# ndming/GS-2M

Measured on AMD Instinct MI355X. Metric: train views/s (fwd+bwd raster) at 1M Gaussians 1080p, higher is better.
Workload: dtype f32; 1 GPU; BASELINE configs[2] (c3): 1000000 synthetic Gaussians (SH deg 3), 1 camera 1920x1080 per GPU, feature_count=9, fwd+bwd at the op boundary; gaussians=1000000, visible=844909, num_rendered=2709460, width=1920, height=1080, feature_count=9, parallelism=view-parallel x1, views_per_rank=1

## Files before the change

### gs-2m_amd/csrc/api.hip

```cpp
#include "raster_args.h"
#include <atomic>
#include <mutex>
#include <chrono>
#include <dlfcn.h>

namespace {

constexpr int kLandSlots = 64, kLandWords = 16;
struct LandRing {
    uint32_t* host = nullptr;
    uint32_t* dev = nullptr;
    std::atomic<uint32_t> next{0};
    std::atomic<uint32_t> gen[kLandSlots];
};
LandRing g_land[64];
std::mutex g_land_mutex;
thread_local uint64_t t_last_token = 0;
thread_local long long t_rows_hint = -1;
thread_local long long t_units_hint = -1, t_units_from_token = -1;

static_assert(GS2M_NUM_STAGES == 10, "stage table");
enum Stage { ST_PREPROCESS = 0, ST_UNUSED1, ST_SCAN, ST_EMIT, ST_TILE_SORT, ST_LISTS, ST_BLEND_FWD, ST_UNUSED7,
             ST_BLEND_BWD, ST_GAUSSIAN_BWD, ST_COUNT };
constexpr int kMaxRecords = 8192;
struct Prof {
    std::atomic<int> mode{0};
    int n = 0;
    hipEvent_t ev[kMaxRecords][2];
    int stage[kMaxRecords];
    int created = 0;
    int every = 1;
    int seen3 = 0;
};
Prof g_prof;
std::mutex g_prof_mutex;
std::atomic<int> g_reference_binning{0};
std::atomic<int> g_spin_wait{1};
std::atomic<int> g_debug{0};
std::atomic<int> g_markers{0};

const char* const kStageNames[ST_COUNT] = {"preprocess", "-", "scan", "emit", "tile_sort", "depth_order+quad_lists", "blend_fwd", "-", "blend_bwd", "gaussian_bwd"};

struct Roctx {
    int (*push)(const char*) = nullptr;
    int (*pop)() = nullptr;
    bool tried = false;
    void load() {
        if (tried) return;
        tried = true;
        void* h = dlopen("libroctx64.so", RTLD_NOW | RTLD_GLOBAL);
        if (!h) h = dlopen("libroctx64.so.4", RTLD_NOW | RTLD_GLOBAL);
        if (!h) return;
        push = (int (*)(const char*))dlsym(h, "roctxRangePushA");
        pop = (int (*)())dlsym(h, "roctxRangePop");
    }
};
Roctx g_roctx;

struct StageTimer {
    hipStream_t s;
    int slot = -1;
    int stage;
    int* failed;
    bool marked = false;
    StageTimer(int stage_, hipStream_t s_, int* failed_ = nullptr) : s(s_), stage(stage_), failed(failed_) {
        if (g_markers.load(std::memory_order_relaxed)) {
            g_roctx.load();
            if (g_roctx.push) { g_roctx.push(kStageNames[stage]); marked = true; }
        }
        const bool blend = stage == ST_BLEND_FWD || stage == ST_BLEND_BWD;
        if (g_prof.mode.load(std::memory_order_relaxed) == 0) return;
        {
            std::lock_guard<std::mutex> lock(g_prof_mutex);
            if (g_prof.mode == 0 || (g_prof.mode == 1 && !blend) || (g_prof.mode == 3 && stage != ST_BLEND_BWD) || g_prof.n >= kMaxRecords) return;
            if (g_prof.mode == 3 && (g_prof.seen3++ % g_prof.every) != 0) return;
            slot = g_prof.n++;
            if (slot >= g_prof.created) {
                (void)hipEventCreate(&g_prof.ev[slot][0]);
                (void)hipEventCreate(&g_prof.ev[slot][1]);
                g_prof.created = slot + 1;
            }
            g_prof.stage[slot] = stage;
        }
        (void)hipEventRecord(g_prof.ev[slot][0], s);
    }
    ~StageTimer() {
        if (slot >= 0) (void)hipEventRecord(g_prof.ev[slot][1], s);
        if (failed && g_debug.load(std::memory_order_relaxed) && *failed == 0) {
            hipError_t e = hipGetLastError();
            if (e == hipSuccess) e = hipStreamSynchronize(s);
            if (e != hipSuccess) *failed = stage + 1;
        }
        if (marked && g_roctx.pop) g_roctx.pop();
    }
};
#define DEBUG_CHECK()                                        \
    do {                                                     \
        if (failed_stage) return GS2M_ERR_STAGE(failed_stage - 1); \
    } while (0)

}

extern "C" {

char* gs2m_prealloc_alloc(size_t bytes, void* user) {
    gs2m_prealloc* p = static_cast<gs2m_prealloc*>(user);
    if (!p) return nullptr;
    p->requested = bytes;
    if (p->ptr && bytes <= p->capacity) return p->ptr;
    p->used_fallback = 1;
    return p->fallback ? p->fallback(bytes, p->fallback_user) : nullptr;
}

const char* gs2m_version(void) { return "gs2m_raster 0.5 (gfx950, round 5)"; }

static int forward_impl(gs2m_alloc_fn geometry_alloc, void* geometry_user, gs2m_alloc_fn binning_alloc, void* binning_user,
                        gs2m_alloc_fn image_alloc, void* image_user, const RasterFrame& f, const float* background, int prefiltered,
                        float* out_color, int* out_radii, int* out_observe, float* out_buffer, void* stream_) {
    hipStream_t s = (hipStream_t)stream_;
    const int reference_binning = g_reference_binning.load(), spin_wait = g_spin_wait.load();
    int failed_stage = 0;
    const unsigned bad = frame_faults(f);
    if (bad & (FRAME_BAD_SHAPE | FRAME_BAD_INPUTS)) return GS2M_ERR_INVALID_ARG;
    if (!geometry_alloc || !binning_alloc || !image_alloc || !out_color || !out_buffer || !background) return GS2M_ERR_INVALID_ARG;
    if (f.P > 0 && (!f.opacities || !out_radii || !out_observe)) return GS2M_ERR_INVALID_ARG;
    if (bad & FRAME_BAD_SPLIT_SH) return GS2M_ERR_UNSUPPORTED;
    if (f.P > 0 && f.fc > 0 && !f.features) return GS2M_ERR_INVALID_ARG;
    if (bad & (FRAME_IMAGE_SIDE | FRAME_TILE_COUNT | FRAME_GAUSSIAN_IDS)) return GS2M_ERR_UNSUPPORTED;
    const int P = f.P, width = f.W, height = f.H, tiles_x = f.tiles_x, tiles_y = f.tiles_y;
    const size_t tiles = (size_t)tiles_x * tiles_y, N = (size_t)width * height;

    const size_t Pn = P > 0 ? (size_t)P : 1;
    GeomState gsz = gs2m_carve_geom(nullptr, Pn);
    char* gbase = geometry_alloc(gsz.total_bytes, geometry_user);
    if (!gbase) return GS2M_ERR_ALLOC;
    GeomState g = gs2m_carve_geom(gbase, Pn);

    ImageState isz = gs2m_carve_image(nullptr, N, tiles);
    char* ibase = image_alloc(isz.total_bytes, image_user);
    if (!ibase) return GS2M_ERR_ALLOC;
    ImageState im = gs2m_carve_image(ibase, N, tiles);

    int dev_id = 0;
    HIP_TRY(hipGetDevice(&dev_id));
    if (dev_id < 0 || dev_id >= 64) return GS2M_ERR_UNSUPPORTED;
    LandRing& ring = g_land[dev_id];
    if (!ring.host) {
        std::lock_guard<std::mutex> lock(g_land_mutex);
        if (!ring.host) {
            uint32_t* h = nullptr;
            HIP_TRY(hipHostMalloc((void**)&h, kLandSlots * kLandWords * sizeof(uint32_t), hipHostMallocMapped | hipHostMallocPortable));
            HIP_TRY(hipHostGetDevicePointer((void**)&ring.dev, h, 0));
            for (int k = 0; k < kLandSlots; k++) ring.gen[k] = 0;
            ring.host = h;
        }
    }
    const uint32_t seq = ring.next.fetch_add(1), slot = seq % kLandSlots;
    const uint32_t generation = ring.gen[slot].fetch_add(1) + 1;
    volatile uint32_t* land = ring.host + slot * kLandWords;
    uint32_t* land_dev = ring.dev + slot * kLandWords;
    land[GS2M_LAND_R] = 0xFFFFFFFFu;
    land[GS2M_LAND_HUNITS] = 0xFFFFFFFFu;
    land[GS2M_LAND_PREFILTERED] = 0u;
    land[GS2M_LAND_ROWS] = 0u;
    t_last_token = ((uint64_t)(dev_id + 1) << 40) | ((uint64_t)(generation & 0xFFFFFFFFu) << 8) | slot;

    int R = 0;
    uint32_t U = 0, crowded = GS2M_CROWDED_WAVE;
    if (P > 0) {
        {
            StageTimer t(ST_PREPROCESS, s, &failed_stage);
            ZeroJobs zj = {{g.tile_hist, nullptr, nullptr}, {(size_t)GS2M_HIST_COPIES * GS2M_HIST_COPY_WORDS, 0, 0}};
            gs2m_launch_preprocess(f, out_radii, out_observe, g, reference_binning ? 0 : 1, zj, s);
        }
        if (prefiltered) gs2m_launch_prefiltered_check(P, f.means3D, f.viewmatrix, land_dev + GS2M_LAND_PREFILTERED, s);
        {
            StageTimer t(ST_SCAN, s, &failed_stage);
            gs2m_launch_blockscan(P, g, land_dev, s);
        }
        HIP_TRY(hipGetLastError());
        DEBUG_CHECK();
        if (spin_wait) {
            const auto t0 = std::chrono::steady_clock::now();
            uint32_t spins = 0;
            while (land[GS2M_LAND_R] == 0xFFFFFFFFu || land[GS2M_LAND_HUNITS] == 0xFFFFFFFFu) {
                __builtin_ia32_pause();
                if ((++spins & 0xFFFFu) == 0u && std::chrono::steady_clock::now() - t0 > std::chrono::seconds(2)) break;
            }
        }
        if (land[GS2M_LAND_R] == 0xFFFFFFFFu || land[GS2M_LAND_HUNITS] == 0xFFFFFFFFu) HIP_TRY(hipStreamSynchronize(s));
        if (prefiltered && land[GS2M_LAND_PREFILTERED] != 0u) {
            HIP_TRY(hipStreamSynchronize(s));
            return GS2M_ERR_PREFILTERED;
        }
        if (land[GS2M_LAND_R] >= (1u << 29)) return GS2M_ERR_UNSUPPORTED;
        R = (int)land[GS2M_LAND_R];
        U = land[GS2M_LAND_HUNITS];
        if ((size_t)U * 4 * GS2M_UNIT > (size_t)6 * (size_t)R + 65536) {
            crowded = GS2M_CROWDED_OFF;
            land[GS2M_LAND_R] = 0xFFFFFFFFu;
            land[GS2M_LAND_HUNITS] = 0xFFFFFFFFu;
            gs2m_launch_recount_heavy(P, g, s);
            gs2m_launch_blockscan(P, g, land_dev, s);
            HIP_TRY(hipGetLastError());
            HIP_TRY(hipStreamSynchronize(s));
            if (land[GS2M_LAND_R] != (uint32_t)R) return GS2M_ERR_STAGE(ST_SCAN);
            U = land[GS2M_LAND_HUNITS];
        }
        if (U >= (1u << 22)) return GS2M_ERR_UNSUPPORTED;
    }

    const int tile_bits = (int)higher_msb((uint32_t)tiles);
    const size_t Rn = R > 0 ? (size_t)R : 1;
    const size_t btemp = gs2m_binning_temp_bytes(Rn, tile_bits);
    BinningState bsz = gs2m_carve_binning(nullptr, Rn, btemp, U);
    char* bbase = binning_alloc(bsz.total_bytes, binning_user);
    if (!bbase) return GS2M_ERR_ALLOC;
    BinningState b = gs2m_carve_binning(bbase, Rn, btemp, U);

    if (R > 0) {
        {
            StageTimer t(ST_EMIT, s, &failed_stage);
            ZeroJobs zj = {{nullptr, im.ranges_raw, nullptr}, {0, tiles * 2, 0}};
            gs2m_radix_zero_region(b.temp, (size_t)R, tile_bits, &zj.p[0], &zj.words[0]);
            gs2m_launch_emit(P, width, height, tiles_x, tile_bits, g, b, U, crowded, land_dev, zj, s);
        }
        if (g_debug.load(std::memory_order_relaxed)) {
            uint32_t total = 0;
            HIP_TRY(hipStreamSynchronize(s));
            HIP_TRY(hipMemcpy(&total, g.counters, sizeof(total), hipMemcpyDeviceToHost));
            if (total != (uint32_t)R) return GS2M_ERR_STAGE(ST_EMIT);
        }
        {
            StageTimer t(ST_TILE_SORT, s, &failed_stage);
            HIP_TRY(gs2m_radix_sort_pairs(b.temp, b.temp_bytes, b.keys_unsorted, nullptr, b.sort_keyA, b.sort_valA, b.tile_keys, b.slot_sorted,
                                          (size_t)R, tile_bits, true, s, im.ranges_raw, g.tile_hist));
        }
    } else {
        HIP_TRY(gs2m_zero_async(im.ranges_raw, tiles * 2 * sizeof(uint32_t), s));
        land[GS2M_LAND_ROWS] = 1u;
        if (land[GS2M_LAND_HUNITS] == 0xFFFFFFFFu) land[GS2M_LAND_HUNITS] = 0u;
    }
    DEBUG_CHECK();
    {
        StageTimer t(ST_LISTS, s, &failed_stage);
        gs2m_launch_tile_sort(tiles, tiles_x, tiles_y, (size_t)(R > 0 ? R : 0), b, im, g, s);
    }
    {
        StageTimer t(ST_BLEND_FWD, s, &failed_stage);
        gs2m_launch_blend_fwd_q(width, height, tiles_x, tiles_y, f.fc, background, g, b, im, out_color, out_buffer, out_observe, s);
    }
    DEBUG_CHECK();
    HIP_TRY(hipGetLastError());
    return R;
}

static int backward_impl(const RasterFrame& f, int R, const float* background, const int* radii, char* geom_buffer, char* binning_buffer,
                         char* image_buffer, const float* grad_colors, const float* grad_buffer, const RasterGrads& d,
                         gs2m_alloc_fn scratch_alloc, void* scratch_user, void* stream_) {
    hipStream_t s = (hipStream_t)stream_;
    int failed_stage = 0;
    if (f.P == 0) return GS2M_OK;
    const unsigned bad = frame_faults(f) | grad_faults(f, d);
    if (bad & FRAME_GAUSSIAN_IDS) return GS2M_ERR_UNSUPPORTED;
    if ((bad & (FRAME_BAD_SHAPE | FRAME_NO_GRADS)) || R < 0) return GS2M_ERR_INVALID_ARG;
    if (!geom_buffer || !binning_buffer || !image_buffer || !scratch_alloc || !grad_colors || !radii) return GS2M_ERR_INVALID_ARG;
    if (f.fc > 0 && !grad_buffer) return GS2M_ERR_INVALID_ARG;
    if (bad & FRAME_BAD_SPLIT_SH) return GS2M_ERR_UNSUPPORTED;
    const int P = f.P, width = f.W, height = f.H, tiles_x = f.tiles_x, tiles_y = f.tiles_y, feature_count = f.fc;
    const size_t tiles = (size_t)tiles_x * tiles_y, N = (size_t)width * height;
    const size_t Rn = R > 0 ? (size_t)R : 1;
    GeomState g = gs2m_carve_geom(geom_buffer, (size_t)P);
    BinningState b = gs2m_carve_binning(binning_buffer, Rn, gs2m_binning_temp_bytes(Rn, (int)higher_msb((uint32_t)tiles)), 0);
    ImageState im = gs2m_carve_image(image_buffer, N, tiles);

    const int rowf = gs2m_row_floats(feature_count);
    const long long hint = t_rows_hint;
    long long units = hint >= 0 ? t_units_hint : -1;
// ... 211 lines not shown
```

### gs-2m_amd/csrc/binning.hip

```cpp
#include "common.h"

GeomState gs2m_carve_geom(char* base, size_t P) {
    GeomState g;
    size_t off = base ? (gs2m_align_up((size_t)(uintptr_t)base) - (size_t)(uintptr_t)base) : 0;
    auto take = [&](size_t bytes) {
        char* p = (char*)((uintptr_t)base + off);
        off = gs2m_align_up(off + bytes);
        return p;
    };
    const size_t nb = (P + 255) / 256 + 1, nw = (P + 63) / 64 + 1;
    g.rec = (float4*)take(P * REC_Q * sizeof(float4));
    g.tiles_touched = (uint32_t*)take(P * 4);
    g.rect = (uint2*)take(P * sizeof(uint2));
    g.depth_key = (uint32_t*)take(P * 4);
    g.clamped = (uint8_t*)take(P);
    g.sh_dir = (float*)take(P * 9 * sizeof(float));
    g.counters = (uint32_t*)take(64 * 4);
    g.gauss_rows = (uint32_t*)take(P * 4);
    g.block_tt = (uint32_t*)take(nb * 4);
    g.block_pref = (uint32_t*)take(nb * 4);
    g.block_hu = (uint32_t*)take(nb * 4);
    g.block_hupref = (uint32_t*)take(nb * 4);
    g.wave_rows = (uint32_t*)take(nw * 4);
    g.wave_rowbase = (uint32_t*)take(nw * 4);
// ... 60 lines not shown
    if (lane == 0) s_part[wave] = v;
    gs2m_sync();
    unsigned long long t = 0;
    for (int w = 0; w < nw; w++) t += s_part[w];
    return t;
}

template <typename F>
__device__ __forceinline__ unsigned long long scan_1024_per_block(const uint32_t* __restrict__ in, size_t n, uint32_t* s_w ,
                                                                  unsigned long long* s_part , F emit) {
    const size_t first = (size_t)blockIdx.x * 1024;
    unsigned long long before = 0;
    for (size_t base = 0; base < first; base += 16 * 1024) {
        uint32_t v[16];
#pragma unroll
        for (int k = 0; k < 16; k++) {
            const size_t i = base + (size_t)k * 1024 + threadIdx.x;
            v[k] = i < first ? in[i] : 0u;
        }
#pragma unroll
        for (int k = 0; k < 16; k++) before += v[k];
    }
    const size_t i = first + threadIdx.x;
    const uint32_t mine = i < n ? in[i] : 0u;
    before = block_sum_u64(before, s_part);
    const int lane = threadIdx.x & 63, wave = threadIdx.x >> 6;
    const uint32_t incl = wave_inclusive_scan_u32(mine, lane);
    if (lane == 63) s_w[wave] = incl;
    gs2m_sync();
    uint32_t run = incl - mine, total = 0;
    for (int w = 0; w < 16; w++) {
        if (w < wave) run += s_w[w];
        total += s_w[w];
    }
    if (i < n) emit(i, (uint32_t)before + run, mine);
    return before + total;
}

template <typename F>
__device__ __forceinline__ void scan2_1024_per_block(const uint32_t* __restrict__ in0, const uint32_t* __restrict__ in1, size_t n, uint32_t* s_w ,
                                                     unsigned long long* s_part , F emit, unsigned long long& total0, unsigned long long& total1) {
    const size_t first = (size_t)blockIdx.x * 1024;
    unsigned long long b0 = 0, b1 = 0;
    for (size_t base = 0; base < first; base += 8 * 1024) {
        uint32_t v[8], w[8];
#pragma unroll
        for (int k = 0; k < 8; k++) {
            const size_t i = base + (size_t)k * 1024 + threadIdx.x;
            v[k] = i < first ? in0[i] : 0u;
            w[k] = i < first ? in1[i] : 0u;
        }
#pragma unroll
        for (int k = 0; k < 8; k++) { b0 += v[k]; b1 += w[k]; }
    }
    const size_t i = first + threadIdx.x;
    const uint32_t m0 = i < n ? in0[i] : 0u, m1 = i < n ? in1[i] : 0u;
    const int lane = threadIdx.x & 63, wave = threadIdx.x >> 6;
#pragma unroll
    for (int d = 32; d > 0; d >>= 1) { b0 += __shfl_xor(b0, d, 64); b1 += __shfl_xor(b1, d, 64); }
    const uint32_t i0 = wave_inclusive_scan_u32(m0, lane), i1 = wave_inclusive_scan_u32(m1, lane);
    if (lane == 0) { s_part[wave] = b0; s_part[16 + wave] = b1; }
    if (lane == 63) { s_w[wave] = i0; s_w[16 + wave] = i1; }
    gs2m_sync();
    unsigned long long f0 = 0, f1 = 0;
    uint32_t r0 = i0 - m0, r1 = i1 - m1, t0 = 0, t1 = 0;
    for (int w = 0; w < 16; w++) {
        f0 += s_part[w]; f1 += s_part[16 + w];
        if (w < wave) { r0 += s_w[w]; r1 += s_w[16 + w]; }
        t0 += s_w[w]; t1 += s_w[16 + w];
    }
    if (i < n) emit(i, (uint32_t)f0 + r0, (uint32_t)f1 + r1);
    total0 = f0 + t0;
    total1 = f1 + t1;
}

__global__ void __launch_bounds__(1024) blockscan_kernel(const uint32_t* __restrict__ block_tt, const uint32_t* __restrict__ block_hu, size_t nblocks,
                                                         uint32_t* __restrict__ block_pref, uint32_t* __restrict__ block_hupref,
                                                         uint32_t* __restrict__ counters, uint32_t* landing) {
    __shared__ uint32_t s_w[32];
    __shared__ unsigned long long s_part[32];
    unsigned long long t = 0, u = 0;
    scan2_1024_per_block(block_tt, block_hu, nblocks, s_w, s_part, [&](size_t b, uint32_t e0, uint32_t e1) { block_pref[b] = e0; block_hupref[b] = e1; }, t, u);
    if (blockIdx.x == gridDim.x - 1 && threadIdx.x == 0) {
        const uint32_t r32 = t > 0xFFFFFFFEull ? 0xFFFFFFFEu : (uint32_t)t, u32 = u > 0xFFFFFFFEull ? 0xFFFFFFFEu : (uint32_t)u;
        __hip_atomic_store(reinterpret_cast<unsigned long long*>(landing + GS2M_LAND_R), (unsigned long long)r32 | ((unsigned long long)u32 << 32),
                           __ATOMIC_RELAXED, __HIP_MEMORY_SCOPE_SYSTEM);
        counters[1] = r32;
        counters[GS2M_CNT_HUNITS] = u32;
        counters[GS2M_CNT_SPAN_MID] = 0u;
        counters[GS2M_CNT_SPAN_LONG] = 0u;
    }
}

__global__ void __launch_bounds__(1024) rowscan_kernel(const uint32_t* __restrict__ wave_rows, size_t nwaves, uint32_t* __restrict__ wave_rowbase,
                                                       uint32_t* __restrict__ counters, uint32_t* landing) {
    __shared__ uint32_t s_w[16];
    __shared__ unsigned long long s_part[16];
    const uint32_t heavy_rows = 4u * GS2M_UNIT * counters[GS2M_CNT_HUNITS];
    const unsigned long long total = heavy_rows + scan_1024_per_block(wave_rows, nwaves, s_w, s_part, [&](size_t w, uint32_t excl, uint32_t) { wave_rowbase[w] = heavy_rows + excl; });
    if (blockIdx.x == gridDim.x - 1 && threadIdx.x == 0) {
        counters[GS2M_CNT_ROWS] = (uint32_t)total;
        publish(landing, GS2M_LAND_ROWS, (uint32_t)total + 1u);
    }
}


__device__ __forceinline__ uint2 expand_instance(uint32_t rmin, uint32_t rwid, uint32_t t, const float4 a , const float2 ct ,
                                                 int W, int H, int tiles_x) {
    const uint32_t ry = t / rwid, rx = t - ry * rwid;
    const uint32_t tx = (rmin & 0xFFFFu) + rx, ty = (rmin >> 16) + ry;
    const int px0 = (int)tx * GS2M_TILE, py0 = (int)ty * GS2M_TILE;
    uint32_t mask = gs2m_reaches_quads(a.x, a.y, a.z, a.w, ct.x, ct.y, (float)px0, (float)py0);
    if (px0 + 8 >= W) mask &= 0x5u;
    if (py0 + 8 >= H) mask &= 0x3u;
    return make_uint2(ty * (uint32_t)tiles_x + tx, mask);
}

__global__ void __launch_bounds__(256) emit_kernel(int P, int W, int H, int tiles_x, const uint2* __restrict__ rect,
                                                   const uint32_t* __restrict__ block_pref, const uint32_t* __restrict__ block_hupref,
                                                   const float4* __restrict__ rec,
                                                   const uint32_t* __restrict__ depth_key, uint32_t* __restrict__ keys_out, uint4* __restrict__ e_rec,
                                                   HeavyUnit* __restrict__ hrec,
                                                   uint32_t* __restrict__ gauss_rows, uint32_t* __restrict__ wave_rows,
                                                   uint32_t* __restrict__ counters, uint32_t* __restrict__ tile_hist, int npass, int4 hbits,
                                                   int4 hshift, uint32_t crowded, ZeroJobs zero) {
    __shared__ uint32_t s_th[4][256];
    __shared__ uint32_t s_pref[4][GS2M_WAVE];
    __shared__ uint32_t s_rmin[4][GS2M_WAVE];
    __shared__ uint32_t s_rw[4][GS2M_WAVE];
    __shared__ uint32_t s_off[4][GS2M_WAVE];
    __shared__ uint32_t s_depth[4][GS2M_WAVE];
    __shared__ float4 s_geo[4][GS2M_WAVE];
    __shared__ float2 s_ct[4][GS2M_WAVE];
    __shared__ uint32_t s_rc[4][GS2M_WAVE];
    __shared__ uint32_t s_wtot[4], s_whu[4];
    const int i = blockIdx.x * 256 + threadIdx.x;
    const int wave = threadIdx.x >> 6, lane = threadIdx.x & 63;
    gs2m_zero_jobs(zero, (size_t)i, (size_t)gridDim.x * 256);
#pragma unroll
    for (int p = 0; p < 4; p++) s_th[p][threadIdx.x] = 0u;
    const int hb[4] = {hbits.x, hbits.y, hbits.z, hbits.w}, hs[4] = {hshift.x, hshift.y, hshift.z, hshift.w};
    uint32_t cnt = 0, rmin = 0, rw = 1;
    if (i < P) {
        const uint2 r = rect[i];
        rmin = r.x;
        rw = r.y & 0xFFFFu;
        cnt = rw * (r.y >> 16);
        if (rw == 0u) rw = 1u;
    }
    const bool heavy = gs2m_heavy(cnt, crowded);
    const uint32_t hu = heavy ? (cnt + GS2M_UNIT - 1u) / GS2M_UNIT : 0u;
    const uint32_t incl_all = wave_inclusive_scan_u32(cnt, lane), incl_hu = wave_inclusive_scan_u32(hu, lane);
    if (lane == 63) { s_wtot[wave] = incl_all; s_whu[wave] = incl_hu; }
    const uint32_t lcnt = heavy ? 0u : cnt;
    if (lcnt > 0) {
        const float4* r = rec + (size_t)i * REC_Q;
        s_geo[wave][lane] = r[REC_GEO0];
        s_ct[wave][lane] = make_float2(r[REC_GEO1].x, r[REC_BIN].w);
        s_depth[wave][lane] = depth_key[i];
    }
    const uint32_t incl = wave_inclusive_scan_u32(lcnt, lane);
    const uint32_t total = __shfl(incl, 63, 64);
    s_pref[wave][lane] = incl - lcnt;
    s_rmin[wave][lane] = rmin;
    s_rw[wave][lane] = rw;
    s_rc[wave][lane] = 0u;
    gs2m_sync();
    uint32_t off = block_pref[blockIdx.x], ustart = block_hupref[blockIdx.x];
#pragma unroll
    for (int w = 0; w < 4; w++)
        if (w < wave) { off += s_wtot[w]; ustart += s_whu[w]; }
// ... 147 lines not shown
```

### gs-2m_amd/csrc/common.h

```cpp
#pragma once
#include <hip/hip_runtime.h>
#include <stdint.h>
#include <stddef.h>
#include "../../include/gs2m_raster.h"

typedef float gs2m_v4f __attribute__((ext_vector_type(4)));
template <typename T> __device__ __forceinline__ T gs2m_ldnt(const T* p) { return __builtin_nontemporal_load(p); }
__device__ __forceinline__ float4 gs2m_ldnt(const float4* p) {
    const gs2m_v4f t = __builtin_nontemporal_load(reinterpret_cast<const gs2m_v4f*>(p));
    return make_float4(t.x, t.y, t.z, t.w);
}
template <typename T> __device__ __forceinline__ void gs2m_stnt(T* p, T v) { __builtin_nontemporal_store(v, p); }
__device__ __forceinline__ void gs2m_stnt(float4* p, float4 v) {
    const gs2m_v4f t = {v.x, v.y, v.z, v.w};
    __builtin_nontemporal_store(t, reinterpret_cast<gs2m_v4f*>(p));
}

#define GS2M_ALIGN 256
#define GS2M_WAVE 64

#define REC_Q 8
#define REC_GEO0 0
#define REC_GEO1 1
#define REC_BIN 2
// ... 105 lines not shown
        }
        const size_t rbase = (size_t)blockIdx.x * 11520, rlim = (size_t)P * 45;
        const bool full = rbase + 11520 <= rlim;
        float4 t[12];
        if (full) {
            const float4* g4 = reinterpret_cast<const float4*>(rest + rbase);
#pragma unroll
            for (int i = 0; i < 11; i++) t[i] = gs2m_ldnt(g4 + tid + 256 * i);
            t[11] = tid < 64 ? gs2m_ldnt(g4 + tid + 2816) : make_float4(0.f, 0.f, 0.f, 0.f);
        } else {
#pragma unroll
            for (int i = 0; i < 12; i++) {
                const int k4 = tid + 256 * i;
                const size_t ge = rbase + 4 * (size_t)k4;
                t[i] = make_float4(0.f, 0.f, 0.f, 0.f);
                if (k4 < 2880) {
                    if (ge + 3 < rlim) {
                        t[i] = *reinterpret_cast<const float4*>(rest + ge);
                    } else {
                        if (ge < rlim) t[i].x = rest[ge];
                        if (ge + 1 < rlim) t[i].y = rest[ge + 1];
                        if (ge + 2 < rlim) t[i].z = rest[ge + 2];
                    }
                }
            }
        }
        int row = (4 * tid) / 45, col = 4 * tid - 45 * row;
#pragma unroll
        for (int i = 0; i < 12; i++) {
            if (i < 11 || tid < 64) {
                const float v[4] = {t[i].x, t[i].y, t[i].z, t[i].w};
                int a = row * 49 + 3 + col, left = 45 - col;
#pragma unroll
                for (int c = 0; c < 4; c++) s_sh[a + c + (c >= left ? 4 : 0)] = v[c];
            }
            row += 22; col += 34;
            if (col >= 45) { col -= 45; row += 1; }
        }
    }
}
#endif

GeomState gs2m_carve_geom(char* base, size_t P);
BinningState gs2m_carve_binning(char* base, size_t R, size_t temp_bytes, size_t heavy_units);
size_t gs2m_binning_temp_bytes(size_t R, int tile_bits);
ImageState gs2m_carve_image(char* base, size_t N, size_t tiles);

size_t gs2m_radix_temp_bytes(size_t n, int total_bits);
hipError_t gs2m_radix_sort_pairs(void* temp, size_t temp_bytes, const uint32_t* kin, const uint32_t* vin, uint32_t* kA,
                                 uint32_t* vA, uint32_t* kB, uint32_t* vB, size_t n, int total_bits, bool prezeroed, hipStream_t s,
                                 uint32_t* range_raw = nullptr, const uint32_t* ext_hist = nullptr);
#define GS2M_HIST_COPIES 8
#define GS2M_HIST_COPY_WORDS 1024
void gs2m_radix_plan(int total_bits, int* npass, int bits[4], int shift[4]);
void gs2m_radix_zero_region(void* temp, size_t n, int total_bits, uint32_t** ptr, size_t* words);

#define GS2M_LAND_R 0
#define GS2M_LAND_HUNITS 1
#define GS2M_LAND_PREFILTERED 2
#define GS2M_LAND_ROWS 3
#define GS2M_CNT_ROWS 2
#define GS2M_CNT_HUNITS 3
#define GS2M_CNT_SPAN_MID 4
#define GS2M_CNT_SPAN_LONG 5

struct RasterFrame {
    int P, D, M, W, H, fc;
    float scale_modifier, tan_fovx, tan_fovy;
    int tiles_x, tiles_y; float focal_x, focal_y;
    const float *means3D, *shs, *shs_rest, *colors_precomp, *opacities, *scales, *rotations, *cov3D_precomp, *features, *viewmatrix, *projmatrix, *cam_pos;
};
static inline RasterFrame gs2m_raster_frame(int W, int H, float tan_fovx, float tan_fovy) {
    RasterFrame f = {};
    f.W = W; f.H = H; f.tan_fovx = tan_fovx; f.tan_fovy = tan_fovy;
    f.tiles_x = W / GS2M_TILE + (W % GS2M_TILE != 0); f.tiles_y = H / GS2M_TILE + (H % GS2M_TILE != 0);
    f.focal_y = H / (2.0f * tan_fovy); f.focal_x = W / (2.0f * tan_fovx);
    return f;
}
struct RasterGrads {
    float *means2D, *conics, *opacities, *colors, *means3D, *cov3D, *shs, *shs_rest, *scales, *rots, *features;
};

void gs2m_launch_preprocess(const RasterFrame& f, int* radii, int* observe_zero, const GeomState& g, int shrink, const ZeroJobs& zero,
                            hipStream_t s);
void gs2m_launch_blockscan(int P, const GeomState& g, uint32_t* landing, hipStream_t s);
void gs2m_launch_rowscan(int P, const GeomState& g, uint32_t* landing, hipStream_t s);
void gs2m_launch_emit(int P, int W, int H, int tiles_x, int tile_bits, const GeomState& g, const BinningState& b, uint32_t heavy_units,
                      uint32_t crowded, uint32_t* landing, const ZeroJobs& zero, hipStream_t s);
void gs2m_launch_recount_heavy(int P, const GeomState& g, hipStream_t s);
void gs2m_launch_heavy_reduce(float* rows, int rowf, const BinningState& b, const GeomState& g, long long heavy_units, hipStream_t s);
void gs2m_set_tile_sort_policy_impl(int policy);
void gs2m_launch_tile_sort(size_t tiles, int tiles_x, int tiles_y, size_t R, const BinningState& b, const ImageState& im, const GeomState& g, hipStream_t s);
hipError_t gs2m_zero_async(void* p, size_t bytes, hipStream_t s);

void gs2m_launch_blend_fwd_q(int W, int H, int tiles_x, int tiles_y, int fc, const float* bg, const GeomState& g,
                             const BinningState& b, const ImageState& im, float* out_color, float* out_buffer,
                             int* out_observe, hipStream_t s);
void gs2m_launch_blend_bwd_q(int W, int H, int tiles_x, int tiles_y, int fc, const float* bg, const GeomState& g,
                             const BinningState& b, const ImageState& im, const float* grad_color,
                             const float* grad_buffer, float* rows, hipStream_t s);
int gs2m_row_floats(int fc);
void gs2m_launch_gaussian_bwd(const RasterFrame& f, const int* radii, const GeomState& g, const float* rows, int rowf, bool have_rows,
                              const RasterGrads& d, hipStream_t s, int force_win = 0);
void gs2m_launch_prefiltered_check(int P, const float* means3D, const float* viewmatrix, uint32_t* flag, hipStream_t s);
void gs2m_launch_mark_visible(int P, const float* means3D, const float* viewmatrix, uint8_t* present, hipStream_t s);

#ifdef __HIPCC__
__device__ __forceinline__ float u2f(uint32_t u) { return __uint_as_float(u); }
__device__ __forceinline__ uint32_t f2u(float f) { return __float_as_uint(f); }

#define DPP_QUAD_PERM(a, b, c, d) ((a) | ((b) << 2) | ((c) << 4) | ((d) << 6))
#define DPP_ROW_HALF_MIRROR 0x141
#define DPP_ROW_MIRROR 0x140

__device__ __forceinline__ void gs2m_sync() {
    asm volatile("s_waitcnt lgkmcnt(0)" ::: "memory");
    __syncthreads();
}
__device__ __forceinline__ int gs2m_sync_or(bool pred) {
    asm volatile("s_waitcnt lgkmcnt(0)" ::: "memory");
    return __syncthreads_or(pred);
}

#define GS2M_CROWDED_OFF 0xFFFFFFFFu
__device__ __forceinline__ bool gs2m_heavy(uint32_t cnt, uint32_t crowded) {
    uint32_t light = cnt < GS2M_HEAVY_TILES ? cnt : 0u;
#pragma unroll
    for (int d = 32; d > 0; d >>= 1) light += (uint32_t)__shfl_xor((int)light, d, 64);
    return cnt >= (light > crowded ? GS2M_HEAVY_TILES_CROWDED : GS2M_HEAVY_TILES) && cnt < (1u << 29);
}

template <typename T>
__device__ __forceinline__ T gs2m_wave_inclusive_scan(T v, int lane) {
#pragma unroll
    for (int d = 1; d < 64; d <<= 1) {
        const T t = __shfl_up(v, d, 64);
        if (lane >= d) v += t;
    }
    return v;
}
__device__ __forceinline__ uint32_t wave_inclusive_scan_u32(uint32_t v, int lane) { return gs2m_wave_inclusive_scan(v, lane); }

template <typename T>
__device__ __forceinline__ T gs2m_wg_exclusive_scan(T v, T* s_w, T* total) {
    const int lane = threadIdx.x & 63, w = threadIdx.x >> 6;
    const T inc = gs2m_wave_inclusive_scan(v, lane);
    if (lane == 63) s_w[w] = inc;
    __syncthreads();
    T off = 0, tot = 0;
#pragma unroll
    for (int k = 0; k < 4; k++) {
        const T x = s_w[k];
        off += k < w ? x : T(0);
        tot += x;
    }
    __syncthreads();
    *total = tot;
    return off + inc - v;
}

#define GS2M_LOG2E 1.4426950408889634f
__device__ __forceinline__ float gs2m_power(float dx, float dy, float A, float B, float C) {
    const float t1 = (A * dx) * dx;
    const float t2 = (C * dy) * dy;
    const float t3 = (B * dx) * dy;
    return (-0.5f * (t1 + t2)) - t3;
}
__device__ __forceinline__ uint32_t gs2m_reaches_quads(float gx, float gy, float A, float B, float C, float t2, float x0, float y0) {
    const float b2 = B + B;
    const float nhrC = -0.5f * __builtin_amdgcn_rcpf(C), nhrA = -0.5f * __builtin_amdgcn_rcpf(A);
    float xl[4], yl[4], blx[4], bly[4], basex[4], basey[4], mx[4], my[4];
#pragma unroll
    for (int i = 0; i < 4; i++) {
        const float o = (float)((i >> 1) * 8 + (i & 1) * 7);
        xl[i] = (x0 + o) - gx; yl[i] = (y0 + o) - gy;
        blx[i] = b2 * xl[i]; bly[i] = b2 * yl[i];
        basex[i] = (A * xl[i]) * xl[i]; basey[i] = (C * yl[i]) * yl[i];
        mx[i] = blx[i] * nhrC;
        my[i] = bly[i] * nhrA;
    }
    uint32_t mask = 0;
#pragma unroll
    for (int q = 0; q < 4; q++) {
        const int qx = q & 1, qy = q >> 1;
        const float lx = xl[2 * qx], ux = xl[2 * qx + 1], ly = yl[2 * qy], uy = yl[2 * qy + 1];
        const bool inside = lx <= 0.f && ux >= 0.f && ly <= 0.f && uy >= 0.f;
        float qe[2];
#pragma unroll
        for (int e = 0; e < 2; e++) {
            const int i = 2 * qx + e;
            const float fm = __builtin_amdgcn_fmed3f(mx[i], ly, uy);
            qe[e] = __builtin_fmaf(__builtin_fmaf(C, fm, blx[i]), fm, basex[i]);
        }
        const float qv = fminf(qe[0], qe[1]);
#pragma unroll
        for (int e = 0; e < 2; e++) {
            const int k = 2 * qy + e;
            const float fm = __builtin_amdgcn_fmed3f(my[k], lx, ux);
            qe[e] = __builtin_fmaf(__builtin_fmaf(A, fm, bly[k]), fm, basey[k]);
        }
        const float qmin = fminf(qv, fminf(qe[0], qe[1]));
        const bool hit = !(t2 < 3.0e38f) || inside || qmin <= __builtin_fmaf(1.0e-3f, fabsf(qmin), t2);
        mask |= hit ? (1u << q) : 0u;
    }
    return mask;
}

__device__ __forceinline__ float gs2m_exp(float x) { return __builtin_amdgcn_exp2f(x * GS2M_LOG2E); }
#endif
```

### gs-2m_amd/csrc/preprocess.hip

```cpp
#include "common.h"
#include "gaussian_math.h"

namespace {

__device__ __forceinline__ int clampi(int v, int lo, int hi) { return min(hi, max(lo, v)); }

template <bool SH_LDS>
__global__ void __launch_bounds__(256) preprocess_kernel(
    int P, int D, int M, const float* __restrict__ means3D, const float* __restrict__ scales, float scale_modifier,
    const float* __restrict__ rotations, const float* __restrict__ opacities, const float* __restrict__ shs,
    const float* __restrict__ shs_rest, const float* __restrict__ cov3D_precomp, const float* __restrict__ colors_precomp,
    const float* __restrict__ features, const float* __restrict__ vm, const float* __restrict__ pm,
    const float* __restrict__ cam_pos, int W, int H, float tan_fovx, float tan_fovy, float focal_x, float focal_y,
    int tiles_x, int tiles_y, int shrink, int* __restrict__ radii, int* __restrict__ observe_zero, float4* __restrict__ rec,
    uint32_t* __restrict__ tiles_touched, uint2* __restrict__ rect, uint32_t* __restrict__ block_tt, uint32_t* __restrict__ block_hu,
    uint32_t* __restrict__ depth_key, uint8_t* __restrict__ clamped, float* __restrict__ sh_dir, ZeroJobs zero) {
    __shared__ __align__(16) float s_sh[SH_LDS ? 256 * 49 : 256 * 45];
    __shared__ uint8_t s_seen[256];
    __shared__ uint32_t s_tt[4];
    __shared__ uint32_t s_hu[4];
    const int idx = blockIdx.x * blockDim.x + threadIdx.x;
    const bool inr = idx < P;
    const int li = inr ? idx : 0;
    const float px = means3D[3 * li], py = means3D[3 * li + 1], pz = means3D[3 * li + 2];
    float in_s[3] = {0.f, 0.f, 0.f};
    float4 in_q = make_float4(0.f, 0.f, 0.f, 0.f);
    if (cov3D_precomp == nullptr) {
        in_s[0] = scales[3 * li]; in_s[1] = scales[3 * li + 1]; in_s[2] = scales[3 * li + 2];
        in_q = reinterpret_cast<const float4*>(rotations)[li];
    }
    const float in_op = opacities[li];
    float2 in_f[GS2M_NUM_FEATURES / 2];
#pragma unroll
    for (int k = 0; k < GS2M_NUM_FEATURES / 2; k++)
        in_f[k] = features != nullptr ? reinterpret_cast<const float2*>(features + (size_t)li * GS2M_NUM_FEATURES)[k] : make_float2(0.f, 0.f);
    if (SH_LDS) {
        gs2m_stage_sh(shs, shs_rest, P, s_sh);
        gs2m_sync();
    }
    gs2m_zero_jobs(zero, (size_t)idx, (size_t)gridDim.x * blockDim.x);
    int out_radius = 0;
    float sd[9] = {0.f, 0.f, 0.f, 0.f, 0.f, 0.f, 0.f, 0.f, 0.f};
    uint32_t out_tt = 0;
    uint32_t out_key = 0xFFFFFFFFu;
    uint2 out_rect = make_uint2(0u, 0u);

    const float3 v = gs2m_view_point(vm, px, py, pz);
    const float vz = v.z;
    float4 rq[REC_Q];
#pragma unroll
    for (int k = 0; k < REC_Q; k++) rq[k] = make_float4(0.f, 0.f, 0.f, 0.f);
    if (inr && vz > kNearZ) {
        const float hx_ = pm[0] * px + pm[4] * py + pm[8] * pz + pm[12];
        const float hy_ = pm[1] * px + pm[5] * py + pm[9] * pz + pm[13];
        const float hw_ = pm[3] * px + pm[7] * py + pm[11] * pz + pm[15];
        const float p_w = 1.0f / (hw_ + 0.0000001f);
        const float projx = hx_ * p_w, projy = hy_ * p_w;

        float c3[6];
        if (cov3D_precomp != nullptr) {
#pragma unroll
            for (int k = 0; k < 6; k++) c3[k] = cov3D_precomp[6 * (size_t)idx + k];
        } else {
            M3 R, Mm;
            gs2m_cov3d(scale_modifier * in_s[0], scale_modifier * in_s[1], scale_modifier * in_s[2], in_q, c3, R, Mm);
        }
        Cov2D pr;
        gs2m_cov2d(v, c3, vm, focal_x, focal_y, tan_fovx, tan_fovy, pr);
        const float cova = pr.cov.m[0][0], covb = pr.cov.m[0][1], covc = pr.cov.m[1][1];
        const float det = cova * covc - covb * covb;
        if (det != 0.0f) {
            const float det_inv = 1.f / det;
            const float cA = covc * det_inv, cB = -covb * det_inv, cC = cova * det_inv;
            const float mid = 0.5f * (cova + covc);
            const float lambda1 = mid + sqrtf(fmaxf(0.1f, mid * mid - det));
            const float lambda2 = mid - sqrtf(fmaxf(0.1f, mid * mid - det));
            const float radius = ceilf(3.f * sqrtf(fmaxf(lambda1, lambda2)));
            const float pix = (float)((((double)projx + 1.0) * (double)W - 1.0) * 0.5);
            const float piy = (float)((((double)projy + 1.0) * (double)H - 1.0) * 0.5);
            const int mr = (int)radius;
            const int rminx = clampi((int)((pix - mr) / GS2M_TILE), 0, tiles_x);
            const int rminy = clampi((int)((piy - mr) / GS2M_TILE), 0, tiles_y);
            const int rmaxx = clampi((int)((pix + mr + GS2M_TILE - 1) / GS2M_TILE), 0, tiles_x);
            const int rmaxy = clampi((int)((piy + mr + GS2M_TILE - 1) / GS2M_TILE), 0, tiles_y);
            const uint32_t rw = (uint32_t)(rmaxx - rminx), rh = (uint32_t)(rmaxy - rminy);
            if (rw * rh != 0) {
                float cr, cg, cb;
                uint8_t cl = 0;
                if (colors_precomp == nullptr) {
                    float dx = px - cam_pos[0], dy = py - cam_pos[1], dz = pz - cam_pos[2];
                    const float len = sqrtf(dx * dx + dy * dy + dz * dz);
                    dx = dx / len; dy = dy / len; dz = dz / len;
                    const float x = dx, y = dy, z = dz;
                    const float* sh = SH_LDS ? (s_sh + threadIdx.x * 49) : (shs + (size_t)idx * M * 3);
                    float res[3];
#pragma unroll
                    for (int c = 0; c < 3; c++) {
                        float r_ = SH_C0 * sh[c];
                        if (D > 0) {
                            r_ = r_ - SH_C1 * y * sh[3 + c] + SH_C1 * z * sh[6 + c] - SH_C1 * x * sh[9 + c];
                            if (D > 1) {
                                const float xx = x * x, yy = y * y, zz = z * z, xy = x * y, yz = y * z, xz = x * z;
                                r_ = r_ + kSH_C2[0] * xy * sh[12 + c] + kSH_C2[1] * yz * sh[15 + c] +
// ... 43 lines not shown
                    }
                } else {
                    cr = colors_precomp[3 * idx]; cg = colors_precomp[3 * idx + 1]; cb = colors_precomp[3 * idx + 2];
                }
                clamped[idx] = cl;

                const float op = in_op;
                float ex, ey;
                float tau2f = __builtin_inff();
                if (op < 1.0f / 255.0f) {
                    ex = ey = -1.0f;
                    tau2f = -1.0f;
                } else {
                    const double dA = cA, dB = cB, dC = cC;
                    const double ddet = dA * dC - dB * dB;
                    if (!(ddet > 0.0) || !(dA > 0.0) || !(dC > 0.0) || dA * dC > 1.0e4 * ddet) {
                        ex = ey = __builtin_inff();
                    } else {
                        const double tau2 = 2.0 * fmax(0.0, log(255.0 * (double)op) + 1.0e-3);
                        ex = (float)(sqrt(tau2 * dC / ddet) * 1.001 + 0.01);
                        ey = (float)(sqrt(tau2 * dA / ddet) * 1.001 + 0.01);
                        tau2f = (float)(tau2 * 1.002 + 1.0e-3);
                    }
                }
                int ex0 = rminx, ex1 = rmaxx, ey0 = rminy, ey1 = rmaxy;
                if (shrink) {
                    if (ex < 0.f) {
                        ex1 = ex0; ey1 = ey0;
                    } else {
                        const float lx = ceilf((pix - ex - 15.0f) * 0.0625f), hx2 = floorf((pix + ex) * 0.0625f) + 1.0f;
                        const float ly = ceilf((piy - ey - 15.0f) * 0.0625f), hy2 = floorf((piy + ey) * 0.0625f) + 1.0f;
                        ex0 = max(ex0, (int)fminf(fmaxf(lx, -1.0f), 70000.0f));
                        ex1 = min(ex1, (int)fminf(fmaxf(hx2, -1.0f), 70000.0f));
                        ey0 = max(ey0, (int)fminf(fmaxf(ly, -1.0f), 70000.0f));
                        ey1 = min(ey1, (int)fminf(fmaxf(hy2, -1.0f), 70000.0f));
                        if (ex1 < ex0) ex1 = ex0;
                        if (ey1 < ey0) ey1 = ey0;
                    }
                }
                const uint32_t ew = (uint32_t)(ex1 - ex0), eh = (uint32_t)(ey1 - ey0);
                float4* r4 = rq;
                r4[REC_GEO0] = make_float4(pix, piy, cA, cB);
                r4[REC_GEO1] = make_float4(cC, op, ex, ey);
                r4[REC_BIN] = make_float4(u2f(0u), u2f((uint32_t)ex0 | ((uint32_t)ey0 << 16)), u2f(ew | (eh << 16)), tau2f);
                float f[GS2M_NUM_FEATURES];
#pragma unroll
                for (int k = 0; k < GS2M_NUM_FEATURES; k++) f[k] = 0.f;
#pragma unroll
                for (int k = 0; k < GS2M_NUM_FEATURES / 2; k++) {
                    f[2 * k] = in_f[k].x; f[2 * k + 1] = in_f[k].y;
                }
                r4[REC_CH + 0] = make_float4(cr, cg, cb, f[0]);
                r4[REC_CH + 1] = make_float4(f[1], f[2], f[3], f[4]);
                r4[REC_CH + 2] = make_float4(f[5], f[6], f[7], f[8]);
                r4[REC_CH + 3] = make_float4(f[9], 0.f, 0.f, 0.f);
                out_radius = mr;
                out_tt = ew * eh;
                if (out_tt != 0u) out_rect = make_uint2((uint32_t)ex0 | ((uint32_t)ey0 << 16), ew | (eh << 16));
                out_key = f2u(vz);
            }
        }
    }
    if (inr) {
        radii[idx] = out_radius;
        if (observe_zero) observe_zero[idx] = 0;
        tiles_touched[idx] = out_tt;
        rect[idx] = out_rect;
        depth_key[idx] = out_key;
    }
    {
        const uint32_t ws = wave_inclusive_scan_u32(out_tt, (int)(threadIdx.x & 63));
        if ((threadIdx.x & 63) == 63) s_tt[threadIdx.x >> 6] = ws;
        uint32_t hu = gs2m_heavy(out_tt, GS2M_CROWDED_WAVE) ? (out_tt + GS2M_UNIT - 1u) / GS2M_UNIT : 0u;
#pragma unroll
        for (int d = 32; d > 0; d >>= 1) hu += __shfl_xor(hu, d, 64);
        if ((threadIdx.x & 63) == 0) s_hu[threadIdx.x >> 6] = hu;
    }
    gs2m_sync();
    float4* s_rec = reinterpret_cast<float4*>(s_sh);
#pragma unroll
    for (int k = 0; k < REC_Q; k++) s_rec[threadIdx.x * 9 + k] = rq[k];
    s_seen[threadIdx.x] = out_radius > 0 ? 1 : 0;
    if (threadIdx.x == 0) {
        block_tt[blockIdx.x] = s_tt[0] + s_tt[1] + s_tt[2] + s_tt[3];
        block_hu[blockIdx.x] = s_hu[0] + s_hu[1] + s_hu[2] + s_hu[3];
    }
    float* s_sd = s_sh + 256 * 36;
    if (colors_precomp == nullptr) {
#pragma unroll
        for (int k = 0; k < 9; k++) s_sd[threadIdx.x * 9 + k] = sd[k];
    }
    gs2m_sync();
    const size_t lim4 = (size_t)P * REC_Q, base4 = (size_t)blockIdx.x * 256 * REC_Q;
#pragma unroll
    for (int k = 0; k < REC_Q; k++) {
        const int e = k * 256 + threadIdx.x;
        if (base4 + e < lim4 && s_seen[e >> 3]) rec[base4 + e] = s_rec[(e >> 3) * 9 + (e & 7)];
    }
    if (colors_precomp == nullptr) {
        const size_t limf = (size_t)P * 9, basef = (size_t)blockIdx.x * 256 * 9;
#pragma unroll
        for (int k = 0; k < 3; k++) {
            const int e4 = k * 256 + threadIdx.x;
            if (e4 < 576) {
                const size_t f0 = basef + 4 * (size_t)e4;
                if (f0 + 3 < limf) {
                    reinterpret_cast<float4*>(sh_dir + basef)[e4] = reinterpret_cast<const float4*>(s_sd)[e4];
                } else {
                    for (int t = 0; t < 4; t++)
                        if (f0 + t < limf) sh_dir[f0 + t] = s_sd[4 * e4 + t];
                }
            }
        }
    }
}

__global__ void mark_visible_kernel(int P, const float* __restrict__ means3D, const float* __restrict__ vm,
                                    uint8_t* __restrict__ present) {
    const int idx = blockIdx.x * blockDim.x + threadIdx.x;
    if (idx >= P) return;
    const float px = means3D[3 * idx], py = means3D[3 * idx + 1], pz = means3D[3 * idx + 2];
    present[idx] = gs2m_view_z(vm, px, py, pz) <= kNearZ ? 0 : 1;
}

__global__ void prefiltered_check_kernel(int P, const float* __restrict__ means3D, const float* __restrict__ vm, uint32_t* flag) {
    const int idx = blockIdx.x * blockDim.x + threadIdx.x;
    bool bad = false;
    if (idx < P) {
        const float px = means3D[3 * idx], py = means3D[3 * idx + 1], pz = means3D[3 * idx + 2];
        bad = !(gs2m_view_z(vm, px, py, pz) > kNearZ);
    }
    if (__builtin_amdgcn_ballot_w64(bad) != 0ull && (threadIdx.x & 63) == 0)
        __hip_atomic_store(flag, 1u, __ATOMIC_RELAXED, __HIP_MEMORY_SCOPE_SYSTEM);
}

}

void gs2m_launch_prefiltered_check(int P, const float* means3D, const float* viewmatrix, uint32_t* flag, hipStream_t s) {
    prefiltered_check_kernel<<<(P + 255) / 256, 256, 0, s>>>(P, means3D, viewmatrix, flag);
}

void gs2m_launch_preprocess(const RasterFrame& f, int* radii, int* observe_zero, const GeomState& g, int shrink, const ZeroJobs& zero,
                            hipStream_t s) {
#define GS2M_PRE(LDS)                                                                                                  \
    preprocess_kernel<LDS><<<(f.P + 255) / 256, 256, 0, s>>>(                                                          \
        f.P, f.D, f.M, f.means3D, f.scales, f.scale_modifier, f.rotations, f.opacities, f.shs, f.shs_rest, f.cov3D_precomp,   \
        f.colors_precomp, f.features, f.viewmatrix, f.projmatrix, f.cam_pos, f.W, f.H, f.tan_fovx, f.tan_fovy, f.focal_x,      \
        f.focal_y, f.tiles_x, f.tiles_y, shrink, radii, observe_zero, g.rec, g.tiles_touched, g.rect, g.block_tt, g.block_hu, \
        g.depth_key, g.clamped, g.sh_dir, zero)
    const bool lds = f.colors_precomp == nullptr && f.shs != nullptr && f.M == 16 &&
                     (f.shs_rest ? (((uintptr_t)f.shs_rest) & 15) == 0 : (((uintptr_t)f.shs) & 15) == 0);
    if (lds) GS2M_PRE(true);
    else GS2M_PRE(false);
#undef GS2M_PRE
}

void gs2m_launch_mark_visible(int P, const float* means3D, const float* viewmatrix, uint8_t* present, hipStream_t s) {
    mark_visible_kernel<<<(P + 255) / 256, 256, 0, s>>>(P, means3D, viewmatrix, present);
}
```

Baseline: 859.4 views/s.

## Publish visible totals from preprocess via last-block ticket reduction

The preprocess kernel now takes an atomic ticket per block, and the last block to finish sums the per-block tile and heavy-unit counts and writes the totals to the host-mapped landing slot. The host therefore sees R and U once preprocess completes instead of after the blockscan kernel, so its spin-wait can end earlier and overlap with the scan. The blockscan no longer publishes to the landing slot. The unfenced ticket path relies on gfx950 write-through cache behaviour, which adds a memory-ordering correctness risk, and the extra reduction lengthens the tail of the preprocess kernel.

```diff
diff --git a/gs-2m_amd/csrc/api.hip b/gs-2m_amd/csrc/api.hip
--- a/gs-2m_amd/csrc/api.hip
+++ b/gs-2m_amd/csrc/api.hip
@@ -6,10 +6,11 @@
 
 namespace {
 
-constexpr int kLandSlots = 64, kLandWords = 16;
+constexpr int kLandSlots = 64, kLandWords = 16, kTicketStride = 32;
 struct LandRing {
     uint32_t* host = nullptr;
     uint32_t* dev = nullptr;
+    uint32_t* tickets = nullptr;
     std::atomic<uint32_t> next{0};
     std::atomic<uint32_t> gen[kLandSlots];
 };
@@ -151,6 +152,8 @@
             uint32_t* h = nullptr;
             HIP_TRY(hipHostMalloc((void**)&h, kLandSlots * kLandWords * sizeof(uint32_t), hipHostMallocMapped | hipHostMallocPortable));
             HIP_TRY(hipHostGetDevicePointer((void**)&ring.dev, h, 0));
+            HIP_TRY(hipMalloc((void**)&ring.tickets, kLandSlots * kTicketStride * sizeof(uint32_t)));
+            HIP_TRY(hipMemset(ring.tickets, 0, kLandSlots * kTicketStride * sizeof(uint32_t)));
             for (int k = 0; k < kLandSlots; k++) ring.gen[k] = 0;
             ring.host = h;
         }
@@ -168,15 +171,15 @@
     int R = 0;
     uint32_t U = 0, crowded = GS2M_CROWDED_WAVE;
     if (P > 0) {
+        if (prefiltered) gs2m_launch_prefiltered_check(P, f.means3D, f.viewmatrix, land_dev + GS2M_LAND_PREFILTERED, s);
         {
             StageTimer t(ST_PREPROCESS, s, &failed_stage);
             ZeroJobs zj = {{g.tile_hist, nullptr, nullptr}, {(size_t)GS2M_HIST_COPIES * GS2M_HIST_COPY_WORDS, 0, 0}};
-            gs2m_launch_preprocess(f, out_radii, out_observe, g, reference_binning ? 0 : 1, zj, s);
-        }
-        if (prefiltered) gs2m_launch_prefiltered_check(P, f.means3D, f.viewmatrix, land_dev + GS2M_LAND_PREFILTERED, s);
+            gs2m_launch_preprocess(f, out_radii, out_observe, g, reference_binning ? 0 : 1, zj, s, ring.tickets + slot * kTicketStride, land_dev);
+        }
         {
             StageTimer t(ST_SCAN, s, &failed_stage);
-            gs2m_launch_blockscan(P, g, land_dev, s);
+            gs2m_launch_blockscan(P, g, nullptr, s);
         }
         HIP_TRY(hipGetLastError());
         DEBUG_CHECK();
@@ -193,7 +196,10 @@
             HIP_TRY(hipStreamSynchronize(s));
             return GS2M_ERR_PREFILTERED;
         }
-        if (land[GS2M_LAND_R] >= (1u << 29)) return GS2M_ERR_UNSUPPORTED;
+        if (land[GS2M_LAND_R] >= (1u << 29)) {
+            HIP_TRY(hipStreamSynchronize(s));
+            return GS2M_ERR_UNSUPPORTED;
+        }
         R = (int)land[GS2M_LAND_R];
         U = land[GS2M_LAND_HUNITS];
         if ((size_t)U * 4 * GS2M_UNIT > (size_t)6 * (size_t)R + 65536) {
diff --git a/gs-2m_amd/csrc/binning.hip b/gs-2m_amd/csrc/binning.hip
--- a/gs-2m_amd/csrc/binning.hip
+++ b/gs-2m_amd/csrc/binning.hip
@@ -166,11 +166,9 @@
     unsigned long long t = 0, u = 0;
     scan2_1024_per_block(block_tt, block_hu, nblocks, s_w, s_part, [&](size_t b, uint32_t e0, uint32_t e1) { block_pref[b] = e0; block_hupref[b] = e1; }, t, u);
     if (blockIdx.x == gridDim.x - 1 && threadIdx.x == 0) {
-        const uint32_t r32 = t > 0xFFFFFFFEull ? 0xFFFFFFFEu : (uint32_t)t, u32 = u > 0xFFFFFFFEull ? 0xFFFFFFFEu : (uint32_t)u;
-        __hip_atomic_store(reinterpret_cast<unsigned long long*>(landing + GS2M_LAND_R), (unsigned long long)r32 | ((unsigned long long)u32 << 32),
-                           __ATOMIC_RELAXED, __HIP_MEMORY_SCOPE_SYSTEM);
-        counters[1] = r32;
-        counters[GS2M_CNT_HUNITS] = u32;
+        const uint2 ru = gs2m_publish_counts(landing, t, u);
+        counters[1] = ru.x;
+        counters[GS2M_CNT_HUNITS] = ru.y;
         counters[GS2M_CNT_SPAN_MID] = 0u;
         counters[GS2M_CNT_SPAN_LONG] = 0u;
     }
diff --git a/gs-2m_amd/csrc/common.h b/gs-2m_amd/csrc/common.h
--- a/gs-2m_amd/csrc/common.h
+++ b/gs-2m_amd/csrc/common.h
@@ -211,7 +211,7 @@
 };
 
 void gs2m_launch_preprocess(const RasterFrame& f, int* radii, int* observe_zero, const GeomState& g, int shrink, const ZeroJobs& zero,
-                            hipStream_t s);
+                            hipStream_t s, uint32_t* ticket = nullptr, uint32_t* landing = nullptr);
 void gs2m_launch_blockscan(int P, const GeomState& g, uint32_t* landing, hipStream_t s);
 void gs2m_launch_rowscan(int P, const GeomState& g, uint32_t* landing, hipStream_t s);
 void gs2m_launch_emit(int P, int W, int H, int tiles_x, int tile_bits, const GeomState& g, const BinningState& b, uint32_t heavy_units,
@@ -335,5 +335,13 @@
     return mask;
 }
 
+__device__ __forceinline__ uint2 gs2m_publish_counts(uint32_t* landing, unsigned long long t, unsigned long long u) {
+    const uint32_t r32 = t > 0xFFFFFFFEull ? 0xFFFFFFFEu : (uint32_t)t, u32 = u > 0xFFFFFFFEull ? 0xFFFFFFFEu : (uint32_t)u;
+    if (landing)
+        __hip_atomic_store(reinterpret_cast<unsigned long long*>(landing + GS2M_LAND_R), (unsigned long long)r32 | ((unsigned long long)u32 << 32),
+                           __ATOMIC_RELAXED, __HIP_MEMORY_SCOPE_SYSTEM);
+    return make_uint2(r32, u32);
+}
+
 __device__ __forceinline__ float gs2m_exp(float x) { return __builtin_amdgcn_exp2f(x * GS2M_LOG2E); }
 #endif
diff --git a/gs-2m_amd/csrc/preprocess.hip b/gs-2m_amd/csrc/preprocess.hip
--- a/gs-2m_amd/csrc/preprocess.hip
+++ b/gs-2m_amd/csrc/preprocess.hip
@@ -14,11 +14,14 @@
     const float* __restrict__ cam_pos, int W, int H, float tan_fovx, float tan_fovy, float focal_x, float focal_y,
     int tiles_x, int tiles_y, int shrink, int* __restrict__ radii, int* __restrict__ observe_zero, float4* __restrict__ rec,
     uint32_t* __restrict__ tiles_touched, uint2* __restrict__ rect, uint32_t* __restrict__ block_tt, uint32_t* __restrict__ block_hu,
-    uint32_t* __restrict__ depth_key, uint8_t* __restrict__ clamped, float* __restrict__ sh_dir, ZeroJobs zero) {
+    uint32_t* __restrict__ depth_key, uint8_t* __restrict__ clamped, float* __restrict__ sh_dir, ZeroJobs zero, uint32_t* ticket,
+    uint32_t* landing) {
     __shared__ __align__(16) float s_sh[SH_LDS ? 256 * 49 : 256 * 45];
     __shared__ uint8_t s_seen[256];
     __shared__ uint32_t s_tt[4];
     __shared__ uint32_t s_hu[4];
+    __shared__ uint32_t s_last;
+    __shared__ unsigned long long s_sum[8];
     const int idx = blockIdx.x * blockDim.x + threadIdx.x;
     const bool inr = idx < P;
     const int li = inr ? idx : 0;
@@ -228,8 +231,8 @@
     for (int k = 0; k < REC_Q; k++) s_rec[threadIdx.x * 9 + k] = rq[k];
     s_seen[threadIdx.x] = out_radius > 0 ? 1 : 0;
     if (threadIdx.x == 0) {
-        block_tt[blockIdx.x] = s_tt[0] + s_tt[1] + s_tt[2] + s_tt[3];
-        block_hu[blockIdx.x] = s_hu[0] + s_hu[1] + s_hu[2] + s_hu[3];
+        __hip_atomic_store(block_tt + blockIdx.x, s_tt[0] + s_tt[1] + s_tt[2] + s_tt[3], __ATOMIC_RELAXED, __HIP_MEMORY_SCOPE_AGENT);
+        __hip_atomic_store(block_hu + blockIdx.x, s_hu[0] + s_hu[1] + s_hu[2] + s_hu[3], __ATOMIC_RELAXED, __HIP_MEMORY_SCOPE_AGENT);
     }
     float* s_sd = s_sh + 256 * 36;
     if (colors_precomp == nullptr) {
@@ -237,6 +240,20 @@
         for (int k = 0; k < 9; k++) s_sd[threadIdx.x * 9 + k] = sd[k];
     }
     gs2m_sync();
+    uint32_t my_ticket = 0u;
+    if (ticket != nullptr && threadIdx.x == 0) {
+#ifdef GS2M_TICKET_FENCED
+        my_ticket = __hip_atomic_fetch_add(ticket, 1u, __ATOMIC_ACQ_REL, __HIP_MEMORY_SCOPE_AGENT);
+#else
+#if defined(__HIP_DEVICE_COMPILE__) && !defined(__gfx950__)
+#error "preprocess_kernel: the unfenced ticket relies on gfx950 cache behaviour (sc1 write-through); build with -DGS2M_TICKET_FENCED elsewhere"
+#endif
+        __atomic_signal_fence(__ATOMIC_SEQ_CST);
+        __builtin_amdgcn_s_waitcnt(0);
+        __atomic_signal_fence(__ATOMIC_SEQ_CST);
+        my_ticket = __hip_atomic_fetch_add(ticket, 1u, __ATOMIC_RELAXED, __HIP_MEMORY_SCOPE_AGENT);
+#endif
+    }
     const size_t lim4 = (size_t)P * REC_Q, base4 = (size_t)blockIdx.x * 256 * REC_Q;
 #pragma unroll
     for (int k = 0; k < REC_Q; k++) {
@@ -259,6 +276,40 @@
             }
         }
     }
+    if (ticket == nullptr) return;
+    if (threadIdx.x == 0) s_last = my_ticket == gridDim.x - 1u ? 1u : 0u;
+    gs2m_sync();
+    if (s_last == 0u) return;
+    const size_t nb = gridDim.x, npair = nb >> 1;
+    const unsigned long long* tt2 = reinterpret_cast<const unsigned long long*>(block_tt);
+    const unsigned long long* hu2 = reinterpret_cast<const unsigned long long*>(block_hu);
+    unsigned long long t = 0, u = 0;
+    for (size_t base = 0; base < npair; base += 8 * 256) {
+        unsigned long long a[8], b[8];
+#pragma unroll
+        for (int k = 0; k < 8; k++) {
+            const size_t i = base + (size_t)k * 256 + threadIdx.x;
+            a[k] = i < npair ? __hip_atomic_load(tt2 + i, __ATOMIC_RELAXED, __HIP_MEMORY_SCOPE_AGENT) : 0ull;
+            b[k] = i < npair ? __hip_atomic_load(hu2 + i, __ATOMIC_RELAXED, __HIP_MEMORY_SCOPE_AGENT) : 0ull;
+        }
+#pragma unroll
+        for (int k = 0; k < 8; k++) {
+            t += (a[k] & 0xFFFFFFFFull) + (a[k] >> 32);
+            u += (b[k] & 0xFFFFFFFFull) + (b[k] >> 32);
+        }
+    }
+    if ((nb & 1) && threadIdx.x == 0) {
+        t += __hip_atomic_load(block_tt + (nb - 1), __ATOMIC_RELAXED, __HIP_MEMORY_SCOPE_AGENT);
+        u += __hip_atomic_load(block_hu + (nb - 1), __ATOMIC_RELAXED, __HIP_MEMORY_SCOPE_AGENT);
+    }
+#pragma unroll
+    for (int d = 32; d > 0; d >>= 1) { t += __shfl_xor(t, d, 64); u += __shfl_xor(u, d, 64); }
+    if ((threadIdx.x & 63) == 0) { s_sum[threadIdx.x >> 6] = t; s_sum[4 + (threadIdx.x >> 6)] = u; }
+    gs2m_sync();
+    if (threadIdx.x == 0) {
+        __hip_atomic_store(ticket, 0u, __ATOMIC_RELAXED, __HIP_MEMORY_SCOPE_AGENT);
+        gs2m_publish_counts(landing, s_sum[0] + s_sum[1] + s_sum[2] + s_sum[3], s_sum[4] + s_sum[5] + s_sum[6] + s_sum[7]);
+    }
 }
 
 __global__ void mark_visible_kernel(int P, const float* __restrict__ means3D, const float* __restrict__ vm,
@@ -287,13 +338,14 @@
 }
 
 void gs2m_launch_preprocess(const RasterFrame& f, int* radii, int* observe_zero, const GeomState& g, int shrink, const ZeroJobs& zero,
-                            hipStream_t s) {
+                            hipStream_t s, uint32_t* ticket, uint32_t* landing) {
+    if (!ticket || !landing) ticket = landing = nullptr;
 #define GS2M_PRE(LDS)                                                                                                  \
     preprocess_kernel<LDS><<<(f.P + 255) / 256, 256, 0, s>>>(                                                          \
         f.P, f.D, f.M, f.means3D, f.scales, f.scale_modifier, f.rotations, f.opacities, f.shs, f.shs_rest, f.cov3D_precomp,   \
         f.colors_precomp, f.features, f.viewmatrix, f.projmatrix, f.cam_pos, f.W, f.H, f.tan_fovx, f.tan_fovy, f.focal_x,      \
         f.focal_y, f.tiles_x, f.tiles_y, shrink, radii, observe_zero, g.rec, g.tiles_touched, g.rect, g.block_tt, g.block_hu, \
-        g.depth_key, g.clamped, g.sh_dir, zero)
+        g.depth_key, g.clamped, g.sh_dir, zero, ticket, landing)
     const bool lds = f.colors_precomp == nullptr && f.shs != nullptr && f.M == 16 &&
                      (f.shs_rest ? (((uintptr_t)f.shs_rest) & 15) == 0 : (((uintptr_t)f.shs) & 15) == 0);
     if (lds) GS2M_PRE(true);
```

Result: no change. 854.7 views/s (-0.5%).
